# piotrkawa/audio-deepfake-adversarial-attacks

Measured on AMD Instinct MI355X. Metric: adversarial utterances/sec, PGD-40 LCNN+LFCC 4s@16kHz, higher is better.
Workload: dtype f32

## Files before the change

### audio_deepfake_adversarial_attacks_amd/_lib.py

```python
from __future__ import annotations

import ctypes
from pathlib import Path

import os

_LIB_PATH = Path(os.environ.get("ADVSTEP_LIB") or Path(__file__).resolve().parent / "libadvstep.so")
_lib = None

OK, EINVAL, EWORKSPACE, ELAUNCH, ENODEVICE = 0, 1, 2, 3, 4
ABI_VERSION = 3

_p, _i64, _f32, _f64, _u64, _sz = (ctypes.c_void_p, ctypes.c_int64, ctypes.c_float, ctypes.c_double,
                                   ctypes.c_uint64, ctypes.c_size_t)

SIGNATURES = {
    "advstep_abi_version": (ctypes.c_int, []),
    "advstep_status_string": (ctypes.c_char_p, [ctypes.c_int]),
    "advstep_device_count": (ctypes.c_int, []),
    "advstep_row_workspace_bytes": (_sz, [_i64, _i64]),
    "advstep_minmax_normalize_f32": (ctypes.c_int, [_p, _p, _p, _p, _i64, _i64, _p, _sz, _p]),
    "advstep_minmax_revert_f32": (ctypes.c_int, [_p, _p, _p, _p, _i64, _i64, _p]),
    "advstep_fgsm_step_f32": (ctypes.c_int, [_p, _p, _p, _i64, _f32, _f32, _f32, _p]),
    "advstep_pgd_linf_init_noise_f32": (ctypes.c_int, [_p, _p, _p, _i64, _f32, _f32, _p]),
# ... 8 lines not shown
    "advstep_cw_tanh_sqdist_f32": (ctypes.c_int, [_p, _p, _p, _p, _i64, _i64, _p, _sz, _p]),
    "advstep_cw_adam_step_f32": (ctypes.c_int, [_p, _p, _p, _p, _p, _i64, _i64, _f64, _f64, _f64, _f64, _p]),
    "advstep_cw_best_update_f32": (ctypes.c_int, [_p, _p, _p, _i64, _i64, _p]),
    "advstep_ce2_loss_grad_f32": (ctypes.c_int, [_p, _p, _p, _p, _i64, _f32, _p]),
    "advstep_mfm_sel_bytes": (_sz, [_i64, _i64, _i64]),
    "advstep_mfm_forward_f32": (ctypes.c_int, [_p, _p, _p, _p, _p, _p, _i64, _i64, _i64, _p]),
    "advstep_mfm_backward_f32": (ctypes.c_int, [_p, _p, _p, _p, _i64, _i64, _i64, _p]),
    "advstep_mfm_pool2_forward_f32": (ctypes.c_int, [_p, _p, _p, _p, _p, _p, _i64, _i64, _i64, _i64, _p]),
    "advstep_mfm_pool2_backward_f32": (ctypes.c_int, [_p, _p, _p, _p, _i64, _i64, _i64, _i64, _p]),
    "advstep_conv5_mfm_pool2_forward_f32": (ctypes.c_int, [_p, _p, _p, _p, _p, _i64, _i64, _i64, _i64, _p]),
    "advstep_conv5_mfm_pool2_backward_f32": (ctypes.c_int, [_p, _p, _p, _p, _i64, _i64, _i64, _i64, _p]),
    "advstep_conv1x1_mfm_supported": (ctypes.c_int, [_i64]),
    "advstep_conv1x1_mfm_sel_bytes": (_sz, [_i64, _i64, _i64]),
    "advstep_conv1x1_mfm_forward_f32": (ctypes.c_int, [_p, _p, _p, _p, _p, _p, _p, _i64, _i64, _i64, _i64, _p]),
    "advstep_conv1x1_mfm_backward_f32": (ctypes.c_int, [_p, _p, _p, _p, _p, _i64, _i64, _i64, _i64, _p]),
    "advstep_lstm_supported": (ctypes.c_int, [_i64]),
    "advstep_lstm_forward_f32": (ctypes.c_int, [_p, _p, _p, _p, _p, _i64, _i64, _i64, _i64, _p]),
    "advstep_lstm_backward_f32": (ctypes.c_int, [_p, _p, _p, _p, _p, _i64, _i64, _i64, _i64, _p]),
    "advstep_lstm_backward_bcast_f32": (ctypes.c_int, [_p, _p, _p, _p, _p, _i64, _i64, _i64, _i64, _p]),
    "advstep_lstm_backward_outer_f32": (ctypes.c_int, [_p, _p, _p, _p, _p, _p, _i64, _i64, _i64, _i64, _p]),
    "advstep_lcnn_tail_pack_f32": (ctypes.c_int, [_p, _p, _i64, _i64, _i64, _i64, _p]),
    "advstep_lcnn_tail_forward_f32": (ctypes.c_int, [_p, _p, _p, _p, _p, _i64, _i64, _i64, _p]),
    "advstep_lcnn_tail_unpack_add_f32": (ctypes.c_int, [_p, _p, _p, _i64, _i64, _i64, _i64, _p]),
    "advstep_lcnn_tail_unpack_add_outer_f32": (ctypes.c_int, [_p, _p, _p, _p, _i64, _i64, _i64, _i64, _p]),
    "advstep_gru_supported": (ctypes.c_int, [_i64]),
    "advstep_gru_forward_f32": (ctypes.c_int, [_p, _p, _p, _p, _p, _i64, _i64, _i64, _i64, _p]),
    "advstep_gru_backward_f32": (ctypes.c_int, [_p, _p, _p, _p, _p, _i64, _i64, _i64, _i64, _p]),
    "advstep_conv3x3_supported": (ctypes.c_int, [_i64, _i64]),
    "advstep_conv3x3_prepared_floats": (_sz, [_i64, _i64, ctypes.c_int]),
    "advstep_conv3x3_prepare_f32": (ctypes.c_int, [_p, _p, _p, _i64, _i64, ctypes.c_int, _p]),
# ... 146 lines not shown
```

### audio_deepfake_adversarial_attacks_amd/csrc/lcnn_conv1x1.hip

```cpp

#include <hip/hip_runtime.h>
#include <math.h>
#include <stdint.h>

#include "advstep_lcnn.h"
#include "advstep_common.h"

namespace {

constexpr int kBlock = 256;
constexpr int kPixPerBlock = 128;

typedef float f32x16 __attribute__((ext_vector_type(16)));

__device__ __forceinline__ int mfma_row(int r, int lane) { return (r & 3) + 8 * (r >> 2) + 4 * (lane >> 5); }

__host__ __device__ constexpr int sel_bit(int s) { return 16 * (s >> 4) + 2 * (s & 1) + 4 * ((s >> 2) & 3); }
__host__ __device__ constexpr int sel_half(int s) { return (s >> 1) & 1; }
inline int64_t sel_mask_bytes(int64_t C) { return C <= 32 ? 2 : 4; }

template <int CIN, int TILES, int MODE>
__global__ __launch_bounds__(kBlock) void conv1x1_mfm_forward_kernel(const float *__restrict__ x,
                                                                     const float *__restrict__ weight,
                                                                     const float *__restrict__ bias,
                                                                     const float *__restrict__ bn_mean,
                                                                     const float *__restrict__ bn_invstd,
                                                                     float *__restrict__ y, uint8_t *__restrict__ sel,
                                                                     int C, int64_t P, int64_t PW) {
    extern __shared__ __attribute__((aligned(16))) float w_s[];
    constexpr int CP = TILES * 32, PITCH = CIN + 1;
    constexpr uint32_t SELB = TILES == 1 ? 2u : 4u;
    float *par_s = w_s + 2 * CP * PITCH;
    constexpr int kWLoads = 2 * CP * CIN / kBlock;
    constexpr int kWBatch = kWLoads % 8 == 0 ? 8 : 12;
    static_assert((2 * CP * CIN) % kBlock == 0 && kWLoads % kWBatch == 0, "weight staging batches");
#pragma unroll
    for (int j0 = 0; j0 < kWLoads; j0 += kWBatch) {
        float wv[kWBatch];
#pragma unroll
        for (int j = 0; j < kWBatch; ++j) {
            const int i = threadIdx.x + (j0 + j) * kBlock, row = i / CIN, ci = i - row * CIN;
            const int half = row / CP, c = row - half * CP;
            wv[j] = weight[(half * C + (c < C ? c : 0)) * CIN + ci];
        }
#pragma unroll
        for (int j = 0; j < kWBatch; ++j) {
            const int i = threadIdx.x + (j0 + j) * kBlock, row = i / CIN, ci = i - row * CIN;
            const int c = row % CP;
            w_s[row * PITCH + ci] = c < C ? wv[j] : 0.0f;
        }
    }
    for (int c = threadIdx.x; c < CP; c += kBlock) {
        const bool live = c < C;
        par_s[c] = (bias && live) ? bias[c] : 0.0f;
        par_s[CP + c] = (bias && live) ? bias[c + C] : 0.0f;
        par_s[2 * CP + c] = (bn_mean && live) ? bn_mean[c] : 0.0f;
        par_s[3 * CP + c] = (bn_mean && live) ? bn_invstd[c] : 1.0f;
    }
    __syncthreads();

    const int64_t n = blockIdx.y;
    const int wave = threadIdx.x >> 6, lane = threadIdx.x & 63, li = lane & 31, lk = lane >> 5;
    const int64_t wave_p0 = ((int64_t)blockIdx.x * 4 + wave) * 32;
    if (wave_p0 >= P) return;
    const int64_t p = wave_p0 + li;
    const bool valid = p < P;
    const uint32_t Pb = (uint32_t)P * 4u;
    const __amdgpu_buffer_rsrc_t xr =
        __builtin_amdgcn_make_buffer_rsrc(const_cast<float *>(x + n * CIN * P), 0, (int)(CIN * Pb), 0x00020000);
    const __amdgpu_buffer_rsrc_t yr = __builtin_amdgcn_make_buffer_rsrc(y + n * (int64_t)C * P, 0, (int)(C * Pb), 0x00020000);
    const __amdgpu_buffer_rsrc_t sr =
        __builtin_amdgcn_make_buffer_rsrc(sel + n * PW * (int64_t)(64u * SELB), 0, (int)((uint32_t)PW * 64u * SELB), 0x00020000);
    constexpr uint32_t kOut = 0x80000000u;
    const uint32_t pb = (uint32_t)p * 4u;
    const uint32_t x_off = valid ? (uint32_t)lk * Pb + pb : kOut;
    const uint32_t y_off = valid ? 4u * (uint32_t)lk * Pb + pb : kOut;
    const uint32_t s_off = valid ? (uint32_t)(2 * li + lk) * SELB : kOut;
    const uint32_t s_tile = (uint32_t)(wave_p0 >> 5) * 64u * SELB;
    uint32_t mask = 0;
    float xb[CIN / 2];
#pragma unroll
    for (int s = 0; s < CIN / 2; ++s)
        xb[s] = __builtin_bit_cast(float, __builtin_amdgcn_raw_buffer_load_b32(xr, x_off, (uint32_t)(2 * s) * Pb, 0));

    constexpr bool FULL = MODE != 0;
    constexpr int kPairTiles = MODE == 2 ? TILES - 1 : TILES;
#pragma unroll
    for (int t = 0; t < kPairTiles; ++t) {
        f32x16 acc_a = {0}, acc_b = {0};
        const float *wa = w_s + (t * 32 + li) * PITCH + lk;
        const float *wb = wa + CP * PITCH;
#pragma unroll
        for (int s = 0; s < CIN / 2; ++s) {
            acc_a = __builtin_amdgcn_mfma_f32_32x32x2f32(wa[2 * s], xb[s], acc_a, 0, 0, 0);
            acc_b = __builtin_amdgcn_mfma_f32_32x32x2f32(wb[2 * s], xb[s], acc_b, 0, 0, 0);
        }
#pragma unroll
        for (int r = 0; r < 16; ++r) {
// ... 20 lines not shown
#pragma unroll
        for (int r = 0; r < 8; ++r) {
            const int c_lo = t * 32 + (r & 3) + 8 * (r >> 2);
            const int c = c_lo + 4 * lk;
            const float va = acc[r] + par_s[c], vb = acc[r + 8] + par_s[CP + c];
            const bool tb = mfm_takes_b(va, vb);
            mask |= tb ? (1u << (16 * t + r)) : 0u;
            const float v = ((tb ? vb : va) - par_s[2 * CP + c]) * par_s[3 * CP + c];
            __builtin_amdgcn_raw_buffer_store_b32(__builtin_bit_cast(uint32_t, v), yr, y_off, (uint32_t)c_lo * Pb, 0);
        }
    }
    if constexpr (SELB == 2) __builtin_amdgcn_raw_buffer_store_b16((uint16_t)mask, sr, s_off, s_tile, 0);
    else __builtin_amdgcn_raw_buffer_store_b32(mask, sr, s_off, s_tile, 0);
}

template <int CIN, int MT, int STEPS>
__global__ __launch_bounds__(kBlock) void conv1x1_mfm_backward_kernel(const float *__restrict__ gy,
                                                                      const uint8_t *__restrict__ sel,
                                                                      const float *__restrict__ weight,
                                                                      const float *__restrict__ gscale,
                                                                      float *__restrict__ gx, int C, int64_t P,
                                                                      int64_t PW) {
    extern __shared__ __attribute__((aligned(16))) float w_s[];
    constexpr int CW = MT * 32, PITCH = CW + 1;
    float *gs_s = w_s + 2 * C * PITCH;
    if constexpr (STEPS > 0) {
        constexpr int kRows = 4 * STEPS, kWLoads = kRows * CW / kBlock, kWBatch = kWLoads % 8 == 0 ? 8 : 12;
        static_assert((kRows * CW) % kBlock == 0 && kWLoads % kWBatch == 0, "weight staging batches");
#pragma unroll
        for (int j0 = 0; j0 < kWLoads; j0 += kWBatch) {
            float wv[kWBatch];
#pragma unroll
            for (int j = 0; j < kWBatch; ++j) {
                const int i = threadIdx.x + (j0 + j) * kBlock, row = i / CW, ci = i - row * CW;
                wv[j] = weight[row * CIN + (ci < CIN ? ci : 0)];
            }
#pragma unroll
            for (int j = 0; j < kWBatch; ++j) {
                const int i = threadIdx.x + (j0 + j) * kBlock, row = i / CW, ci = i - row * CW;
                w_s[row * PITCH + ci] = ci < CIN ? wv[j] : 0.0f;
            }
        }
    } else {
        for (int i = threadIdx.x; i < 2 * C * CW; i += kBlock) {
            const int row = i / CW, ci = i - row * CW;
            w_s[row * PITCH + ci] = ci < CIN ? weight[(int64_t)row * CIN + ci] : 0.0f;
        }
    }
    for (int c = threadIdx.x; c < C; c += kBlock) gs_s[c] = gscale ? gscale[c] : 1.0f;
    __syncthreads();

    const int64_t n = blockIdx.y;
    const int wave = threadIdx.x >> 6, lane = threadIdx.x & 63, li = lane & 31, lk = lane >> 5;
    const int64_t p = (int64_t)blockIdx.x * kPixPerBlock + wave * 32 + li;
    const bool valid = p < P;
    if ((int64_t)blockIdx.x * kPixPerBlock + wave * 32 >= P) return;

    const uint32_t Pb = (uint32_t)P * 4u;
    const bool wide = C > 32;
    const uint32_t pairb = wide ? 8u : 4u;
    const __amdgpu_buffer_rsrc_t gr =
        __builtin_amdgcn_make_buffer_rsrc(const_cast<float *>(gy + n * (int64_t)C * P), 0, (int)(C * Pb), 0x00020000);
    const __amdgpu_buffer_rsrc_t sr = __builtin_amdgcn_make_buffer_rsrc(
        const_cast<uint8_t *>(sel + n * PW * (int64_t)(32u * pairb)), 0, (int)((uint32_t)PW * 32u * pairb), 0x00020000);
    const __amdgpu_buffer_rsrc_t xr = __builtin_amdgcn_make_buffer_rsrc(gx + n * CIN * P, 0, (int)(CIN * Pb), 0x00020000);
    constexpr uint32_t kOut = 0x80000000u;
    const uint32_t pb = (uint32_t)p * 4u;
    const uint32_t g_off = valid ? (uint32_t)lk * Pb + pb : kOut;
    const uint32_t x_off = valid ? 4u * (uint32_t)lk * Pb + pb : kOut;
    const uint32_t s_off = valid ? (uint32_t)li * pairb : kOut;
    const uint32_t s_tile = (uint32_t)(((int64_t)blockIdx.x * kPixPerBlock + wave * 32) >> 5) * 32u * pairb;
    uint32_t m[2];
    if (wide) {
        m[0] = __builtin_amdgcn_raw_buffer_load_b32(sr, s_off, s_tile, 0) >> lk;
        m[1] = __builtin_amdgcn_raw_buffer_load_b32(sr, s_off + (valid ? 4u : 0u), s_tile, 0) >> lk;
    } else {
        const uint32_t both = __builtin_amdgcn_raw_buffer_load_b32(sr, s_off, s_tile, 0);
        m[0] = (both & 0xffffu) >> lk;
        m[1] = (both >> 16) >> lk;
    }
    f32x16 acc[MT];
#pragma unroll
    for (int m = 0; m < MT; ++m) acc[m] = (f32x16){0};
    if constexpr (STEPS > 0) {
        float g[STEPS];
#pragma unroll
        for (int s = 0; s < STEPS; ++s)
            g[s] = __builtin_bit_cast(float, __builtin_amdgcn_raw_buffer_load_b32(gr, g_off, (uint32_t)(2 * s) * Pb, 0));
#pragma unroll
        for (int s = 0; s < STEPS; ++s) {
            const int c = 2 * s + lk;
            const float gs = g[s] * gs_s[c];
            const bool tb = (m[sel_half(s)] >> sel_bit(s)) & 1u;
            const float ga = tb ? 0.0f : gs, gb = tb ? gs : 0.0f;
            const float *wa = w_s + c * PITCH + li;
            const float *wb = wa + C * PITCH;
#pragma unroll
            for (int m = 0; m < MT; ++m) {
                acc[m] = __builtin_amdgcn_mfma_f32_32x32x2f32(wa[32 * m], ga, acc[m], 0, 0, 0);
                acc[m] = __builtin_amdgcn_mfma_f32_32x32x2f32(wb[32 * m], gb, acc[m], 0, 0, 0);
            }
        }
    } else {
    const int steps = (C + 1) >> 1;
    for (int s = 0; s < steps; ++s) {
        const int c = 2 * s + lk;
        const bool live = c < C;
        const float g = live ? __builtin_bit_cast(float, __builtin_amdgcn_raw_buffer_load_b32(gr, g_off, (uint32_t)(2 * s) * Pb, 0)) *
                                   gs_s[c]
                             : 0.0f;
        const bool tb = live && ((m[sel_half(s)] >> sel_bit(s)) & 1u);
        const float ga = tb ? 0.0f : g, gb = tb ? g : 0.0f;
        const float *wa = w_s + (live ? c : 0) * PITCH + li;
        const float *wb = w_s + ((live ? c : 0) + C) * PITCH + li;
#pragma unroll
        for (int m = 0; m < MT; ++m) {
            acc[m] = __builtin_amdgcn_mfma_f32_32x32x2f32(live ? wa[32 * m] : 0.0f, ga, acc[m], 0, 0, 0);
            acc[m] = __builtin_amdgcn_mfma_f32_32x32x2f32(live ? wb[32 * m] : 0.0f, gb, acc[m], 0, 0, 0);
// ... 8 lines not shown
            static_assert(CIN % 8 == 0, "row pairs (ci, ci + 4) must be live or dead together");
            const float gv = acc[m][r];
            if (ci_lo < CIN)
                __builtin_amdgcn_raw_buffer_store_b32(__float_as_uint(gv), xr, x_off, (uint32_t)ci_lo * Pb, 0);
        }
    }
}

template <typename K>
void opt_in_lds(K kernel, size_t bytes) {
    if (bytes > 48 * 1024)
        (void)hipFuncSetAttribute(reinterpret_cast<const void *>(kernel), hipFuncAttributeMaxDynamicSharedMemorySize,
                                  (int)bytes);
}

template <int CIN, int TILES>
void launch_fwd(const float *x, const float *w, const float *b, const float *bn_mean, const float *bn_invstd, float *y,
                uint8_t *sel, int64_t N, int64_t C, int64_t P, hipStream_t st) {
    const size_t lds = (size_t)(2 * TILES * 32 * (CIN + 1) + 4 * TILES * 32) * sizeof(float);
    const dim3 grid((unsigned)ceil_div(P, kPixPerBlock), (unsigned)N);
    if (C == TILES * 32) {
        opt_in_lds(conv1x1_mfm_forward_kernel<CIN, TILES, 1>, lds);
        hipLaunchKernelGGL((conv1x1_mfm_forward_kernel<CIN, TILES, 1>), grid, dim3(kBlock), lds, st, x, w, b, bn_mean,
                           bn_invstd, y, sel, (int)C, P, ceil_div(P, 32));
    } else if (C == TILES * 32 - 16) {
        opt_in_lds(conv1x1_mfm_forward_kernel<CIN, TILES, 2>, lds);
        hipLaunchKernelGGL((conv1x1_mfm_forward_kernel<CIN, TILES, 2>), grid, dim3(kBlock), lds, st, x, w, b, bn_mean,
                           bn_invstd, y, sel, (int)C, P, ceil_div(P, 32));
    } else {
        opt_in_lds(conv1x1_mfm_forward_kernel<CIN, TILES, 0>, lds);
        hipLaunchKernelGGL((conv1x1_mfm_forward_kernel<CIN, TILES, 0>), grid, dim3(kBlock), lds, st, x, w, b, bn_mean,
                           bn_invstd, y, sel, (int)C, P, ceil_div(P, 32));
    }
}

template <int CIN, int MT, int STEPS>
void launch_bwd_steps(const float *gy, const uint8_t *sel, const float *w, const float *gscale, float *gx, int64_t N,
                      int64_t C, int64_t P, hipStream_t st) {
    const size_t lds = (size_t)(2 * C * (MT * 32 + 1) + C) * sizeof(float);
    opt_in_lds(conv1x1_mfm_backward_kernel<CIN, MT, STEPS>, lds);
    const dim3 grid((unsigned)ceil_div(P, kPixPerBlock), (unsigned)N);
    hipLaunchKernelGGL((conv1x1_mfm_backward_kernel<CIN, MT, STEPS>), grid, dim3(kBlock), lds, st, gy, sel, w, gscale, gx,
                       (int)C, P, ceil_div(P, 32));
}

template <int CIN, int MT>
void launch_bwd(const float *gy, const uint8_t *sel, const float *w, const float *gscale, float *gx, int64_t N, int64_t C,
                int64_t P, hipStream_t st) {
    if (C == CIN)
        launch_bwd_steps<CIN, MT, CIN / 2>(gy, sel, w, gscale, gx, N, C, P, st);
    else
        launch_bwd_steps<CIN, MT, 0>(gy, sel, w, gscale, gx, N, C, P, st);
}

}

extern "C" {

int advstep_conv1x1_mfm_supported(int64_t Cin) { return Cin == 32 || Cin == 48 || Cin == 64; }

size_t advstep_conv1x1_mfm_sel_bytes(int64_t N, int64_t C, int64_t P) {
    if (N <= 0 || C <= 0 || P <= 0) return 0;
    return (size_t)N * (size_t)ceil_div(P, 32) * 64u * (size_t)sel_mask_bytes(C);
}

int advstep_conv1x1_mfm_forward_f32(const float *x, const float *weight, const float *bias, const float *bn_mean,
                                    const float *bn_invstd, float *y, void *sel, int64_t N, int64_t Cin, int64_t C,
                                    int64_t P, advstep_stream_t stream) {
    ADVSTEP_REQUIRE(N >= 0 && C >= 0 && P >= 0 && advstep_conv1x1_mfm_supported(Cin));
    if (N == 0 || C == 0 || P == 0) return ADVSTEP_OK;
    ADVSTEP_REQUIRE(x && weight && y && sel && N <= kMaxGridY && C <= 64 && ((reinterpret_cast<uintptr_t>(sel) & 3u) == 0));
    ADVSTEP_REQUIRE((bn_mean == nullptr) == (bn_invstd == nullptr));
    auto *s32 = static_cast<uint8_t *>(sel);
    hipStream_t st = as_stream(stream);
    const bool two = C > 32;
    switch (Cin) {
        case 32:
            two ? launch_fwd<32, 2>(x, weight, bias, bn_mean, bn_invstd, y, s32, N, C, P, st)
                : launch_fwd<32, 1>(x, weight, bias, bn_mean, bn_invstd, y, s32, N, C, P, st);
            break;
        case 48:
            two ? launch_fwd<48, 2>(x, weight, bias, bn_mean, bn_invstd, y, s32, N, C, P, st)
                : launch_fwd<48, 1>(x, weight, bias, bn_mean, bn_invstd, y, s32, N, C, P, st);
            break;
        default:
            two ? launch_fwd<64, 2>(x, weight, bias, bn_mean, bn_invstd, y, s32, N, C, P, st)
                : launch_fwd<64, 1>(x, weight, bias, bn_mean, bn_invstd, y, s32, N, C, P, st);
            break;
    }
    return status_after_launch();
}

int advstep_conv1x1_mfm_backward_f32(const float *gy, const void *sel, const float *weight, const float *gscale, float *gx,
                                     int64_t N, int64_t Cin, int64_t C, int64_t P, advstep_stream_t stream) {
    ADVSTEP_REQUIRE(N >= 0 && C >= 0 && P >= 0 && advstep_conv1x1_mfm_supported(Cin));
    if (N == 0 || P == 0) return ADVSTEP_OK;
    ADVSTEP_REQUIRE(gx && N <= kMaxGridY && C <= 64);
    hipStream_t st = as_stream(stream);
    if (C == 0)
        return hipMemsetAsync(gx, 0, (size_t)N * Cin * P * sizeof(float), st) == hipSuccess ? ADVSTEP_OK : ADVSTEP_ELAUNCH;
    ADVSTEP_REQUIRE(gy && sel && weight);
    ADVSTEP_REQUIRE((reinterpret_cast<uintptr_t>(sel) & 3u) == 0);
    auto *s32 = static_cast<const uint8_t *>(sel);
    switch (Cin) {
        case 32: launch_bwd<32, 1>(gy, s32, weight, gscale, gx, N, C, P, st); break;
        case 48: launch_bwd<48, 2>(gy, s32, weight, gscale, gx, N, C, P, st); break;
        default: launch_bwd<64, 2>(gy, s32, weight, gscale, gx, N, C, P, st); break;
    }
    return status_after_launch();
}

}
```

### audio_deepfake_adversarial_attacks_amd/lcnn_ops.py

```python
from __future__ import annotations

from typing import Optional

import torch

from . import _lib
from .hip_ops import _Launch, _require, _stream


def _gemm(fn, a2d: torch.Tensor, b2d: torch.Tensor, *lead):
    with _Launch("rnn_projection_gemm", a2d.device, work=2.0 * a2d.shape[0] * a2d.shape[1] * b2d.shape[1]):
        return fn(*lead, a2d, b2d)


def _check_input(x: torch.Tensor, bias: Optional[torch.Tensor]):
    _require(x, "x")
    if x.dim() != 4 or x.shape[1] % 2 != 0:
        raise ValueError(f"expected a contiguous (N, 2C, H, W) tensor, got {tuple(x.shape)}")
    if bias is not None:
        _require(bias, "bias")
        if bias.numel() != x.shape[1]:
            raise ValueError(f"bias must have {x.shape[1]} entries, got {bias.numel()}")


# ... 106 lines not shown
        idx, weight = ctx.saved_tensors
        N, C, H, W = ctx.shape
        gy = gy.contiguous()
        gx = torch.empty((N, 1, H, W), dtype=gy.dtype, device=gy.device)
        with _Launch("conv5_mfm_pool2_backward", gy.device, work=12.5 * N * C * H * W, tensors=(gy, idx, gx)):
            st = _lib.load().advstep_conv5_mfm_pool2_backward_f32(gy.data_ptr(), idx.data_ptr(), weight.data_ptr(),
                                                                  gx.data_ptr(), N, C, H, W, _stream(gy.device))
        _lib.check(st, "advstep_conv5_mfm_pool2_backward_f32")
        return gx, None, None


def conv5_mfm_pool2(x: torch.Tensor, weight: torch.Tensor, bias: Optional[torch.Tensor] = None) -> torch.Tensor:
    return _Conv5MfmPool2.apply(x.contiguous(), weight.contiguous(), bias)


class _Conv1x1Mfm(torch.autograd.Function):

    @staticmethod
    def forward(ctx, x, weight, bias, bn):
        _require(x, "x"), _require(weight, "weight")
        if bias is not None:
            _require(bias, "bias")
        bn_mean, bn_invstd = _bn_ptrs(bn)
        if x.dim() != 4 or weight.dim() != 4 or tuple(weight.shape[2:]) != (1, 1) or weight.shape[1] != x.shape[1] \
                or weight.shape[0] % 2 != 0 or (bias is not None and bias.numel() != weight.shape[0]):
            raise ValueError(f"expected x (N, Cin, H, W), weight (2C, Cin, 1, 1), bias (2C); got {tuple(x.shape)}, "
                             f"{tuple(weight.shape)}")
        N, Cin, H, W = x.shape
        C, P = weight.shape[0] // 2, H * W
        lib = _lib.load()
        if not lib.advstep_conv1x1_mfm_supported(Cin):
            raise ValueError(f"conv1x1_mfm supports Cin in (32, 48, 64), got {Cin}")
        y = torch.empty((N, C, H, W), dtype=x.dtype, device=x.device)
        sel = torch.empty(max(lib.advstep_conv1x1_mfm_sel_bytes(N, C, P), 4), dtype=torch.uint8, device=x.device)
        with _Launch("conv1x1_mfm_forward", x.device, work=4.0 * N * Cin * C * P, tensors=(x, y, sel)):
            st = lib.advstep_conv1x1_mfm_forward_f32(x.data_ptr(), weight.data_ptr(),
                                                     bias.data_ptr() if bias is not None else None, bn_mean, bn_invstd,
                                                     y.data_ptr(), sel.data_ptr(), N, Cin, C, P, _stream(x.device))
        _lib.check(st, "advstep_conv1x1_mfm_forward_f32")
        ctx.save_for_backward(sel, weight, *([bn[1]] if bn is not None else []))
        ctx.shape = (N, Cin, C, H, W)
        return y

    @staticmethod
    def backward(ctx, gy):
        if ctx.needs_input_grad[1] or (len(ctx.needs_input_grad) > 2 and ctx.needs_input_grad[2]):
            raise RuntimeError("conv1x1_mfm provides the input gradient only; call it with frozen weights "
                               "(the model falls back to Conv2d + mfm otherwise)")
        sel, weight, *scale = ctx.saved_tensors
        N, Cin, C, H, W = ctx.shape
        gy = gy.contiguous()
        gx = torch.empty((N, Cin, H, W), dtype=gy.dtype, device=gy.device)
        with _Launch("conv1x1_mfm_backward", gy.device, work=4.0 * N * Cin * C * H * W, tensors=(gy, sel, gx)):
            st = _lib.load().advstep_conv1x1_mfm_backward_f32(gy.data_ptr(), sel.data_ptr(), weight.data_ptr(),
                                                              scale[0].data_ptr() if scale else None, gx.data_ptr(), N, Cin,
                                                              C, H * W, _stream(gy.device))
        _lib.check(st, "advstep_conv1x1_mfm_backward_f32")
        return gx, None, None, None


def conv1x1_mfm_supported(in_channels: int) -> bool:
    return bool(_lib.load().advstep_conv1x1_mfm_supported(in_channels))


def conv1x1_mfm(x: torch.Tensor, weight: torch.Tensor, bias: Optional[torch.Tensor] = None, bn=None) -> torch.Tensor:
    return _Conv1x1Mfm.apply(x.contiguous(), weight.contiguous(), bias, bn)



def _prepared_weights(weight: torch.Tensor, mode: int, gscale: Optional[torch.Tensor] = None) -> torch.Tensor:
    cache = getattr(weight, "_advstep_wino", None)
    if cache is None or cache[0] != (weight._version, weight.data_ptr()):
        cache = ((weight._version, weight.data_ptr()), {})
        try:
            weight._advstep_wino = cache
        except AttributeError:
            pass
    slot = (mode, None if gscale is None else (gscale.data_ptr(), gscale._version))
    U = cache[1].get(slot)
    if U is None:
        Cout, Cin = weight.shape[0], weight.shape[1]
# ... 326 lines not shown
```

### include/advstep_lcnn.h

```cpp
#ifndef ADVSTEP_LCNN_H_
#define ADVSTEP_LCNN_H_

#include <stddef.h>
#include <stdint.h>

#include "advstep.h"

#ifdef __cplusplus
extern "C" {
#endif

size_t advstep_mfm_sel_bytes(int64_t N, int64_t C, int64_t HW);

int advstep_mfm_forward_f32(const float *x, const float *bias, const float *bn_mean, const float *bn_invstd, float *y,
                            uint8_t *sel, int64_t N, int64_t C, int64_t HW, advstep_stream_t stream);

int advstep_mfm_backward_f32(const float *gy, const uint8_t *sel, const float *gscale, float *gx, int64_t N, int64_t C,
                             int64_t HW, advstep_stream_t stream);

int advstep_mfm_pool2_forward_f32(const float *x, const float *bias, const float *bn_mean, const float *bn_invstd,
                                  float *y, uint8_t *idx, int64_t N, int64_t C, int64_t H, int64_t W,
                                  advstep_stream_t stream);

int advstep_mfm_pool2_backward_f32(const float *gy, const uint8_t *idx, const float *gscale, float *gx, int64_t N,
// ... 1 lines not shown

int advstep_conv5_mfm_pool2_forward_f32(const float *x, const float *weight, const float *bias, float *y, uint8_t *idx,
                                        int64_t N, int64_t C, int64_t H, int64_t W, advstep_stream_t stream);

int advstep_conv5_mfm_pool2_backward_f32(const float *gy, const uint8_t *idx, const float *weight, float *gx, int64_t N,
                                         int64_t C, int64_t H, int64_t W, advstep_stream_t stream);

int advstep_conv1x1_mfm_supported(int64_t Cin);
size_t advstep_conv1x1_mfm_sel_bytes(int64_t N, int64_t C, int64_t P);
int advstep_conv1x1_mfm_forward_f32(const float *x, const float *weight, const float *bias, const float *bn_mean,
                                    const float *bn_invstd, float *y, void *sel, int64_t N, int64_t Cin, int64_t C,
                                    int64_t P, advstep_stream_t stream);

int advstep_conv1x1_mfm_backward_f32(const float *gy, const void *sel, const float *weight, const float *gscale,
                                     float *gx, int64_t N, int64_t Cin, int64_t C, int64_t P, advstep_stream_t stream);

int advstep_conv3x3_supported(int64_t Cin, int64_t Cout);
size_t advstep_conv3x3_prepared_floats(int64_t Cin, int64_t Cout, int mode);
int advstep_conv3x3_prepare_f32(const float *weight, const float *gscale, float *U, int64_t Cin, int64_t Cout, int mode,
                                advstep_stream_t stream);

int advstep_conv3x3_mfm_pool2_forward_f32(const float *x, const float *U, const float *bias, const float *bn_mean,
                                          const float *bn_invstd, float *y, uint8_t *idx, int64_t N, int64_t Cin,
                                          int64_t C, int64_t H, int64_t W, advstep_stream_t stream);

size_t advstep_conv3x3_mfm_sel_bytes(int64_t N, int64_t C, int64_t H, int64_t W);
int advstep_conv3x3_mfm_forward_f32(const float *x, const float *U, const float *bias, const float *bn_mean,
                                    const float *bn_invstd, float *y, uint8_t *sel, int64_t N, int64_t Cin, int64_t C,
                                    int64_t H, int64_t W, advstep_stream_t stream);
int advstep_conv3x3_mfm_backward_f32(const float *gy, const uint8_t *sel, const float *gscale, float *gout, int64_t N,
// ... 38 lines not shown
```

Measured before the change: 2040.

## Prepare padded conv1x1 weight images and stream them into LDS asynchronously

Adds a one-time prepare step that packs conv1x1 weights, bias, BN params and grad scales into a padded LDS-ready image. The image is cached on the frozen weight tensor. The forward and backward kernels then copy that image with global_load_lds DMA, which overlaps with their activation loads and replaces per-block strided weight staging through registers. The trade-offs are a host-side cache keyed on tensor version and pointer, extra template variants, and early-exit wave returns being dropped so every wave reaches the barrier.

After: 2048, median of 6. Within noise of the previous version (+0.4%).

```diff
diff --git a/audio_deepfake_adversarial_attacks_amd/_lib.py b/audio_deepfake_adversarial_attacks_amd/_lib.py
--- a/audio_deepfake_adversarial_attacks_amd/_lib.py
+++ b/audio_deepfake_adversarial_attacks_amd/_lib.py
@@ -46,6 +46,11 @@
     "advstep_conv1x1_mfm_sel_bytes": (_sz, [_i64, _i64, _i64]),
     "advstep_conv1x1_mfm_forward_f32": (ctypes.c_int, [_p, _p, _p, _p, _p, _p, _p, _i64, _i64, _i64, _i64, _p]),
     "advstep_conv1x1_mfm_backward_f32": (ctypes.c_int, [_p, _p, _p, _p, _p, _i64, _i64, _i64, _i64, _p]),
+    "advstep_conv1x1_mfm_prepared_floats": (_sz, [_i64, _i64, ctypes.c_int]),
+    "advstep_conv1x1_mfm_prepared_preferred": (ctypes.c_int, [_i64, _i64, ctypes.c_int]),
+    "advstep_conv1x1_mfm_prepare_f32": (ctypes.c_int, [_p, _p, _p, _p, _p, _i64, _i64, ctypes.c_int, _p]),
+    "advstep_conv1x1_mfm_forward_prepared_f32": (ctypes.c_int, [_p, _p, _p, _p, _i64, _i64, _i64, _i64, _p]),
+    "advstep_conv1x1_mfm_backward_prepared_f32": (ctypes.c_int, [_p, _p, _p, _p, _i64, _i64, _i64, _i64, _p]),
     "advstep_lstm_supported": (ctypes.c_int, [_i64]),
     "advstep_lstm_forward_f32": (ctypes.c_int, [_p, _p, _p, _p, _p, _i64, _i64, _i64, _i64, _p]),
     "advstep_lstm_backward_f32": (ctypes.c_int, [_p, _p, _p, _p, _p, _i64, _i64, _i64, _i64, _p]),
diff --git a/audio_deepfake_adversarial_attacks_amd/csrc/lcnn_conv1x1.hip b/audio_deepfake_adversarial_attacks_amd/csrc/lcnn_conv1x1.hip
--- a/audio_deepfake_adversarial_attacks_amd/csrc/lcnn_conv1x1.hip
+++ b/audio_deepfake_adversarial_attacks_amd/csrc/lcnn_conv1x1.hip
@@ -19,7 +19,78 @@
 __host__ __device__ constexpr int sel_half(int s) { return (s >> 1) & 1; }
 inline int64_t sel_mask_bytes(int64_t C) { return C <= 32 ? 2 : 4; }
 
-template <int CIN, int TILES, int MODE>
+__host__ __device__ constexpr int fwd_image_floats(int CIN, int TILES) { return 2 * TILES * 32 * (CIN + 1) + 4 * TILES * 32; }
+__host__ __device__ constexpr int bwd_image_floats(int C, int MT) { return (2 * C * (32 * MT + 1) + C + 3) & ~3; }
+__host__ __device__ constexpr int image_lds_bytes(int floats) { return ((floats / 4 + 63) & ~63) * 16; }
+
+template <int N4>
+__device__ __forceinline__ void image_to_lds(const float *__restrict__ image, float *lds, int n4_runtime) {
+    const float4 *src = reinterpret_cast<const float4 *>(image);
+    float4 *dst = reinterpret_cast<float4 *>(lds);
+    const int n4 = N4 > 0 ? N4 : n4_runtime;
+    const int w64 = __builtin_amdgcn_readfirstlane((int)(threadIdx.x >> 6) << 6), lane = threadIdx.x & 63;
+    if constexpr (N4 > 0) {
+#pragma unroll
+        for (int i = 0; i < (N4 + kBlock - 1) / kBlock; ++i) {
+            const int base = w64 + i * kBlock;
+            if (i * kBlock + kBlock - 64 < N4 || base < N4)
+                __builtin_amdgcn_global_load_lds((const __attribute__((address_space(1))) void *)(src + min(base + lane, N4 - 1)),
+                                                 (__attribute__((address_space(3))) void *)(dst + base), 16, 0, 0);
+        }
+    } else {
+        for (int base = w64; base < n4; base += kBlock)
+            __builtin_amdgcn_global_load_lds((const __attribute__((address_space(1))) void *)(src + min(base + lane, n4 - 1)),
+                                             (__attribute__((address_space(3))) void *)(dst + base), 16, 0, 0);
+    }
+    __builtin_amdgcn_sched_barrier(0);
+}
+template <int LATER>
+__device__ __forceinline__ void image_landed_barrier() {
+    static_assert(LATER >= 0 && LATER < 64, "vmcnt is a 6-bit counter");
+    __builtin_amdgcn_s_waitcnt((LATER & 15) | 0x0F70 | ((LATER >> 4) << 14));
+    __builtin_amdgcn_s_barrier();
+}
+
+__global__ __launch_bounds__(kBlock) void conv1x1_prepare_forward_kernel(const float *__restrict__ weight,
+                                                                         const float *__restrict__ bias,
+                                                                         const float *__restrict__ bn_mean,
+                                                                         const float *__restrict__ bn_invstd,
+                                                                         float *__restrict__ image, int CIN, int C, int CP) {
+    const int PITCH = CIN + 1, nw = 2 * CP * PITCH, n = nw + 4 * CP;
+    for (int i = blockIdx.x * kBlock + threadIdx.x; i < n; i += gridDim.x * kBlock) {
+        float v;
+        if (i < nw) {
+            const int row = i / PITCH, ci = i - row * PITCH, half = row / CP, c = row - half * CP;
+            v = (c < C && ci < CIN) ? weight[(half * C + c) * CIN + ci] : 0.0f;
+        } else {
+            const int j = i - nw, k = j / CP, c = j - k * CP;
+            const bool live = c < C;
+            if (k < 2) v = (bias && live) ? bias[c + k * C] : 0.0f;
+            else if (k == 2) v = (bn_mean && live) ? bn_mean[c] : 0.0f;
+            else v = (bn_mean && live) ? bn_invstd[c] : 1.0f;
+        }
+        image[i] = v;
+    }
+}
+
+__global__ __launch_bounds__(kBlock) void conv1x1_prepare_backward_kernel(const float *__restrict__ weight,
+                                                                          const float *__restrict__ gscale,
+                                                                          float *__restrict__ image, int CIN, int C, int CW,
+                                                                          int n) {
+    const int PITCH = CW + 1, nw = 2 * C * PITCH;
+    for (int i = blockIdx.x * kBlock + threadIdx.x; i < n; i += gridDim.x * kBlock) {
+        float v = 0.0f;
+        if (i < nw) {
+            const int row = i / PITCH, ci = i - row * PITCH;
+            v = ci < CIN ? weight[row * CIN + ci] : 0.0f;
+        } else if (i < nw + C) {
+            v = gscale ? gscale[i - nw] : 1.0f;
+        }
+        image[i] = v;
+    }
+}
+
+template <int CIN, int TILES, int MODE, bool PREP>
 __global__ __launch_bounds__(kBlock) void conv1x1_mfm_forward_kernel(const float *__restrict__ x,
                                                                      const float *__restrict__ weight,
                                                                      const float *__restrict__ bias,
@@ -34,6 +105,7 @@
     constexpr int kWLoads = 2 * CP * CIN / kBlock;
     constexpr int kWBatch = kWLoads % 8 == 0 ? 8 : 12;
     static_assert((2 * CP * CIN) % kBlock == 0 && kWLoads % kWBatch == 0, "weight staging batches");
+    if constexpr (!PREP) {
 #pragma unroll
     for (int j0 = 0; j0 < kWLoads; j0 += kWBatch) {
         float wv[kWBatch];
@@ -58,11 +130,16 @@
         par_s[3 * CP + c] = (bn_mean && live) ? bn_invstd[c] : 1.0f;
     }
     __syncthreads();
+    } else {
+        static_assert(fwd_image_floats(CIN, TILES) % 4 == 0, "the image is a whole number of float4");
+        image_to_lds<fwd_image_floats(CIN, TILES) / 4>(weight, w_s, 0);
+    }
 
     const int64_t n = blockIdx.y;
-    const int wave = threadIdx.x >> 6, lane = threadIdx.x & 63, li = lane & 31, lk = lane >> 5;
+    const int wave = PREP ? __builtin_amdgcn_readfirstlane((int)(threadIdx.x >> 6)) : (int)(threadIdx.x >> 6);
+    const int lane = threadIdx.x & 63, li = lane & 31, lk = lane >> 5;
     const int64_t wave_p0 = ((int64_t)blockIdx.x * 4 + wave) * 32;
-    if (wave_p0 >= P) return;
+    if (!PREP && wave_p0 >= P) return;
     const int64_t p = wave_p0 + li;
     const bool valid = p < P;
     const uint32_t Pb = (uint32_t)P * 4u;
@@ -82,6 +159,7 @@
 #pragma unroll
     for (int s = 0; s < CIN / 2; ++s)
         xb[s] = __builtin_bit_cast(float, __builtin_amdgcn_raw_buffer_load_b32(xr, x_off, (uint32_t)(2 * s) * Pb, 0));
+    if constexpr (PREP) image_landed_barrier<CIN / 2>();
 
     constexpr bool FULL = MODE != 0;
     constexpr int kPairTiles = MODE == 2 ? TILES - 1 : TILES;
@@ -132,7 +210,7 @@
     else __builtin_amdgcn_raw_buffer_store_b32(mask, sr, s_off, s_tile, 0);
 }
 
-template <int CIN, int MT, int STEPS>
+template <int CIN, int MT, int STEPS, bool PREP>
 __global__ __launch_bounds__(kBlock) void conv1x1_mfm_backward_kernel(const float *__restrict__ gy,
                                                                       const uint8_t *__restrict__ sel,
                                                                       const float *__restrict__ weight,
@@ -142,7 +220,10 @@
     extern __shared__ __attribute__((aligned(16))) float w_s[];
     constexpr int CW = MT * 32, PITCH = CW + 1;
     float *gs_s = w_s + 2 * C * PITCH;
-    if constexpr (STEPS > 0) {
+    if constexpr (PREP) {
+        if constexpr (STEPS > 0) image_to_lds<bwd_image_floats(2 * STEPS, MT) / 4>(weight, w_s, 0);
+        else image_to_lds<0>(weight, w_s, bwd_image_floats(C, MT) / 4);
+    } else if constexpr (STEPS > 0) {
         constexpr int kRows = 4 * STEPS, kWLoads = kRows * CW / kBlock, kWBatch = kWLoads % 8 == 0 ? 8 : 12;
         static_assert((kRows * CW) % kBlock == 0 && kWLoads % kWBatch == 0, "weight staging batches");
 #pragma unroll
@@ -165,17 +246,20 @@
             w_s[row * PITCH + ci] = ci < CIN ? weight[(int64_t)row * CIN + ci] : 0.0f;
         }
     }
+    if constexpr (!PREP) {
     for (int c = threadIdx.x; c < C; c += kBlock) gs_s[c] = gscale ? gscale[c] : 1.0f;
     __syncthreads();
+    }
 
     const int64_t n = blockIdx.y;
-    const int wave = threadIdx.x >> 6, lane = threadIdx.x & 63, li = lane & 31, lk = lane >> 5;
+    const int wave = PREP ? __builtin_amdgcn_readfirstlane((int)(threadIdx.x >> 6)) : (int)(threadIdx.x >> 6);
+    const int lane = threadIdx.x & 63, li = lane & 31, lk = lane >> 5;
     const int64_t p = (int64_t)blockIdx.x * kPixPerBlock + wave * 32 + li;
     const bool valid = p < P;
-    if ((int64_t)blockIdx.x * kPixPerBlock + wave * 32 >= P) return;
+    if (!PREP && (int64_t)blockIdx.x * kPixPerBlock + wave * 32 >= P) return;
 
     const uint32_t Pb = (uint32_t)P * 4u;
-    const bool wide = C > 32;
+    const bool wide = (PREP && STEPS > 0) ? STEPS > 16 : C > 32;
     const uint32_t pairb = wide ? 8u : 4u;
     const __amdgpu_buffer_rsrc_t gr =
         __builtin_amdgcn_make_buffer_rsrc(const_cast<float *>(gy + n * (int64_t)C * P), 0, (int)(C * Pb), 0x00020000);
@@ -205,6 +289,7 @@
 #pragma unroll
         for (int s = 0; s < STEPS; ++s)
             g[s] = __builtin_bit_cast(float, __builtin_amdgcn_raw_buffer_load_b32(gr, g_off, (uint32_t)(2 * s) * Pb, 0));
+        if constexpr (PREP) image_landed_barrier<STEPS + (STEPS > 16 ? 2 : 1)>();
 #pragma unroll
         for (int s = 0; s < STEPS; ++s) {
             const int c = 2 * s + lk;
@@ -220,6 +305,7 @@
             }
         }
     } else {
+    if constexpr (PREP) image_landed_barrier<0>();
     const int steps = (C + 1) >> 1;
     for (int s = 0; s < steps; ++s) {
         const int c = 2 * s + lk;
@@ -258,44 +344,75 @@
                                   (int)bytes);
 }
 
-template <int CIN, int TILES>
+template <int CIN, int TILES, bool PREP>
 void launch_fwd(const float *x, const float *w, const float *b, const float *bn_mean, const float *bn_invstd, float *y,
                 uint8_t *sel, int64_t N, int64_t C, int64_t P, hipStream_t st) {
-    const size_t lds = (size_t)(2 * TILES * 32 * (CIN + 1) + 4 * TILES * 32) * sizeof(float);
+    const size_t lds = PREP ? (size_t)image_lds_bytes(fwd_image_floats(CIN, TILES))
+                            : (size_t)(2 * TILES * 32 * (CIN + 1) + 4 * TILES * 32) * sizeof(float);
     const dim3 grid((unsigned)ceil_div(P, kPixPerBlock), (unsigned)N);
     if (C == TILES * 32) {
-        opt_in_lds(conv1x1_mfm_forward_kernel<CIN, TILES, 1>, lds);
-        hipLaunchKernelGGL((conv1x1_mfm_forward_kernel<CIN, TILES, 1>), grid, dim3(kBlock), lds, st, x, w, b, bn_mean,
+        opt_in_lds(conv1x1_mfm_forward_kernel<CIN, TILES, 1, PREP>, lds);
+        hipLaunchKernelGGL((conv1x1_mfm_forward_kernel<CIN, TILES, 1, PREP>), grid, dim3(kBlock), lds, st, x, w, b, bn_mean,
                            bn_invstd, y, sel, (int)C, P, ceil_div(P, 32));
     } else if (C == TILES * 32 - 16) {
-        opt_in_lds(conv1x1_mfm_forward_kernel<CIN, TILES, 2>, lds);
-        hipLaunchKernelGGL((conv1x1_mfm_forward_kernel<CIN, TILES, 2>), grid, dim3(kBlock), lds, st, x, w, b, bn_mean,
+        opt_in_lds(conv1x1_mfm_forward_kernel<CIN, TILES, 2, PREP>, lds);
+        hipLaunchKernelGGL((conv1x1_mfm_forward_kernel<CIN, TILES, 2, PREP>), grid, dim3(kBlock), lds, st, x, w, b, bn_mean,
                            bn_invstd, y, sel, (int)C, P, ceil_div(P, 32));
     } else {
-        opt_in_lds(conv1x1_mfm_forward_kernel<CIN, TILES, 0>, lds);
-        hipLaunchKernelGGL((conv1x1_mfm_forward_kernel<CIN, TILES, 0>), grid, dim3(kBlock), lds, st, x, w, b, bn_mean,
+        opt_in_lds(conv1x1_mfm_forward_kernel<CIN, TILES, 0, PREP>, lds);
+        hipLaunchKernelGGL((conv1x1_mfm_forward_kernel<CIN, TILES, 0, PREP>), grid, dim3(kBlock), lds, st, x, w, b, bn_mean,
                            bn_invstd, y, sel, (int)C, P, ceil_div(P, 32));
     }
 }
 
-template <int CIN, int MT, int STEPS>
+template <int CIN, bool PREP>
+void launch_fwd_tiles(const float *x, const float *w, const float *b, const float *bn_mean, const float *bn_invstd, float *y,
+                      uint8_t *sel, int64_t N, int64_t C, int64_t P, hipStream_t st) {
+    C > 32 ? launch_fwd<CIN, 2, PREP>(x, w, b, bn_mean, bn_invstd, y, sel, N, C, P, st)
+           : launch_fwd<CIN, 1, PREP>(x, w, b, bn_mean, bn_invstd, y, sel, N, C, P, st);
+}
+
+template <bool PREP>
+void launch_fwd_cin(const float *x, const float *w, const float *b, const float *bn_mean, const float *bn_invstd, float *y,
+                    uint8_t *sel, int64_t N, int64_t Cin, int64_t C, int64_t P, hipStream_t st) {
+    switch (Cin) {
+        case 32: launch_fwd_tiles<32, PREP>(x, w, b, bn_mean, bn_invstd, y, sel, N, C, P, st); break;
+        case 48: launch_fwd_tiles<48, PREP>(x, w, b, bn_mean, bn_invstd, y, sel, N, C, P, st); break;
+        default: launch_fwd_tiles<64, PREP>(x, w, b, bn_mean, bn_invstd, y, sel, N, C, P, st); break;
+    }
+}
+
+template <int CIN, int MT, int STEPS, bool PREP>
 void launch_bwd_steps(const float *gy, const uint8_t *sel, const float *w, const float *gscale, float *gx, int64_t N,
                       int64_t C, int64_t P, hipStream_t st) {
-    const size_t lds = (size_t)(2 * C * (MT * 32 + 1) + C) * sizeof(float);
-    opt_in_lds(conv1x1_mfm_backward_kernel<CIN, MT, STEPS>, lds);
+    const size_t lds = PREP ? (size_t)image_lds_bytes(bwd_image_floats((int)C, MT))
+                            : (size_t)(2 * C * (MT * 32 + 1) + C) * sizeof(float);
+    opt_in_lds(conv1x1_mfm_backward_kernel<CIN, MT, STEPS, PREP>, lds);
     const dim3 grid((unsigned)ceil_div(P, kPixPerBlock), (unsigned)N);
-    hipLaunchKernelGGL((conv1x1_mfm_backward_kernel<CIN, MT, STEPS>), grid, dim3(kBlock), lds, st, gy, sel, w, gscale, gx,
-                       (int)C, P, ceil_div(P, 32));
-}
-
-template <int CIN, int MT>
+    hipLaunchKernelGGL((conv1x1_mfm_backward_kernel<CIN, MT, STEPS, PREP>), grid, dim3(kBlock), lds, st, gy, sel, w, gscale,
+                       gx, (int)C, P, ceil_div(P, 32));
+}
+
+template <int CIN, int MT, bool PREP>
 void launch_bwd(const float *gy, const uint8_t *sel, const float *w, const float *gscale, float *gx, int64_t N, int64_t C,
                 int64_t P, hipStream_t st) {
     if (C == CIN)
-        launch_bwd_steps<CIN, MT, CIN / 2>(gy, sel, w, gscale, gx, N, C, P, st);
+        launch_bwd_steps<CIN, MT, CIN / 2, PREP>(gy, sel, w, gscale, gx, N, C, P, st);
     else
-        launch_bwd_steps<CIN, MT, 0>(gy, sel, w, gscale, gx, N, C, P, st);
-}
+        launch_bwd_steps<CIN, MT, 0, PREP>(gy, sel, w, gscale, gx, N, C, P, st);
+}
+
+template <bool PREP>
+void launch_bwd_cin(const float *gy, const uint8_t *sel, const float *w, const float *gscale, float *gx, int64_t N,
+                    int64_t Cin, int64_t C, int64_t P, hipStream_t st) {
+    switch (Cin) {
+        case 32: launch_bwd<32, 1, PREP>(gy, sel, w, gscale, gx, N, C, P, st); break;
+        case 48: launch_bwd<48, 2, PREP>(gy, sel, w, gscale, gx, N, C, P, st); break;
+        default: launch_bwd<64, 2, PREP>(gy, sel, w, gscale, gx, N, C, P, st); break;
+    }
+}
+
+inline int mt_of(int64_t Cin) { return Cin > 32 ? 2 : 1; }
 
 }
 
@@ -315,23 +432,7 @@
     if (N == 0 || C == 0 || P == 0) return ADVSTEP_OK;
     ADVSTEP_REQUIRE(x && weight && y && sel && N <= kMaxGridY && C <= 64 && ((reinterpret_cast<uintptr_t>(sel) & 3u) == 0));
     ADVSTEP_REQUIRE((bn_mean == nullptr) == (bn_invstd == nullptr));
-    auto *s32 = static_cast<uint8_t *>(sel);
-    hipStream_t st = as_stream(stream);
-    const bool two = C > 32;
-    switch (Cin) {
-        case 32:
-            two ? launch_fwd<32, 2>(x, weight, bias, bn_mean, bn_invstd, y, s32, N, C, P, st)
-                : launch_fwd<32, 1>(x, weight, bias, bn_mean, bn_invstd, y, s32, N, C, P, st);
-            break;
-        case 48:
-            two ? launch_fwd<48, 2>(x, weight, bias, bn_mean, bn_invstd, y, s32, N, C, P, st)
-                : launch_fwd<48, 1>(x, weight, bias, bn_mean, bn_invstd, y, s32, N, C, P, st);
-            break;
-        default:
-            two ? launch_fwd<64, 2>(x, weight, bias, bn_mean, bn_invstd, y, s32, N, C, P, st)
-                : launch_fwd<64, 1>(x, weight, bias, bn_mean, bn_invstd, y, s32, N, C, P, st);
-            break;
-    }
+    launch_fwd_cin<false>(x, weight, bias, bn_mean, bn_invstd, y, static_cast<uint8_t *>(sel), N, Cin, C, P, as_stream(stream));
     return status_after_launch();
 }
 
@@ -345,13 +446,62 @@
         return hipMemsetAsync(gx, 0, (size_t)N * Cin * P * sizeof(float), st) == hipSuccess ? ADVSTEP_OK : ADVSTEP_ELAUNCH;
     ADVSTEP_REQUIRE(gy && sel && weight);
     ADVSTEP_REQUIRE((reinterpret_cast<uintptr_t>(sel) & 3u) == 0);
-    auto *s32 = static_cast<const uint8_t *>(sel);
-    switch (Cin) {
-        case 32: launch_bwd<32, 1>(gy, s32, weight, gscale, gx, N, C, P, st); break;
-        case 48: launch_bwd<48, 2>(gy, s32, weight, gscale, gx, N, C, P, st); break;
-        default: launch_bwd<64, 2>(gy, s32, weight, gscale, gx, N, C, P, st); break;
-    }
+    launch_bwd_cin<false>(gy, static_cast<const uint8_t *>(sel), weight, gscale, gx, N, Cin, C, P, st);
     return status_after_launch();
 }
 
-}
+size_t advstep_conv1x1_mfm_prepared_floats(int64_t Cin, int64_t C, int direction) {
+    if (!advstep_conv1x1_mfm_supported(Cin) || C <= 0 || C > 64 || (direction != 0 && direction != 1)) return 0;
+    return direction == 0 ? (size_t)fwd_image_floats((int)Cin, C > 32 ? 2 : 1) : (size_t)bwd_image_floats((int)C, mt_of(Cin));
+}
+
+int advstep_conv1x1_mfm_prepared_preferred(int64_t Cin, int64_t C, int direction) {
+    if (advstep_conv1x1_mfm_prepared_floats(Cin, C, direction) == 0) return 0;
+    if (Cin == 48 && C == 48) return 1;
+    return Cin == 32 && C == 32 && direction == 1;
+}
+
+int advstep_conv1x1_mfm_prepare_f32(const float *weight, const float *bias, const float *bn_mean, const float *scale,
+                                    float *image, int64_t Cin, int64_t C, int direction, advstep_stream_t stream) {
+    ADVSTEP_REQUIRE(C >= 0 && C <= 64 && advstep_conv1x1_mfm_supported(Cin) && (direction == 0 || direction == 1));
+    if (C == 0) return ADVSTEP_OK;
+    ADVSTEP_REQUIRE(weight && image && aligned16(image));
+    const int n = (int)advstep_conv1x1_mfm_prepared_floats(Cin, C, direction);
+    const dim3 grid((unsigned)ceil_div(n, 4 * kBlock));
+    if (direction == 0) {
+        ADVSTEP_REQUIRE((bn_mean == nullptr) == (scale == nullptr));
+        hipLaunchKernelGGL(conv1x1_prepare_forward_kernel, grid, dim3(kBlock), 0, as_stream(stream), weight, bias, bn_mean, scale,
+                           image, (int)Cin, (int)C, C > 32 ? 64 : 32);
+    } else {
+        ADVSTEP_REQUIRE(bias == nullptr && bn_mean == nullptr);
+        hipLaunchKernelGGL(conv1x1_prepare_backward_kernel, grid, dim3(kBlock), 0, as_stream(stream), weight, scale, image,
+                           (int)Cin, (int)C, 32 * mt_of(Cin), n);
+    }
+    return status_after_launch();
+}
+
+int advstep_conv1x1_mfm_forward_prepared_f32(const float *x, const float *image, float *y, void *sel, int64_t N, int64_t Cin,
+                                             int64_t C, int64_t P, advstep_stream_t stream) {
+    ADVSTEP_REQUIRE(N >= 0 && C >= 0 && P >= 0 && advstep_conv1x1_mfm_supported(Cin));
+    if (N == 0 || C == 0 || P == 0) return ADVSTEP_OK;
+    ADVSTEP_REQUIRE(x && image && aligned16(image) && y && sel && N <= kMaxGridY && C <= 64 &&
+                    ((reinterpret_cast<uintptr_t>(sel) & 3u) == 0));
+    launch_fwd_cin<true>(x, image, nullptr, nullptr, nullptr, y, static_cast<uint8_t *>(sel), N, Cin, C, P, as_stream(stream));
+    return status_after_launch();
+}
+
+int advstep_conv1x1_mfm_backward_prepared_f32(const float *gy, const void *sel, const float *image, float *gx, int64_t N,
+                                              int64_t Cin, int64_t C, int64_t P, advstep_stream_t stream) {
+    ADVSTEP_REQUIRE(N >= 0 && C >= 0 && P >= 0 && advstep_conv1x1_mfm_supported(Cin));
+    if (N == 0 || P == 0) return ADVSTEP_OK;
+    ADVSTEP_REQUIRE(gx && N <= kMaxGridY && C <= 64);
+    hipStream_t st = as_stream(stream);
+    if (C == 0)
+        return hipMemsetAsync(gx, 0, (size_t)N * Cin * P * sizeof(float), st) == hipSuccess ? ADVSTEP_OK : ADVSTEP_ELAUNCH;
+    ADVSTEP_REQUIRE(gy && sel && image && aligned16(image));
+    ADVSTEP_REQUIRE((reinterpret_cast<uintptr_t>(sel) & 3u) == 0);
+    launch_bwd_cin<true>(gy, static_cast<const uint8_t *>(sel), image, nullptr, gx, N, Cin, C, P, st);
+    return status_after_launch();
+}
+
+}
diff --git a/audio_deepfake_adversarial_attacks_amd/lcnn_ops.py b/audio_deepfake_adversarial_attacks_amd/lcnn_ops.py
--- a/audio_deepfake_adversarial_attacks_amd/lcnn_ops.py
+++ b/audio_deepfake_adversarial_attacks_amd/lcnn_ops.py
@@ -1,5 +1,6 @@
 from __future__ import annotations
 
+import os
 from typing import Optional
 
 import torch
@@ -144,31 +145,72 @@
     return _Conv5MfmPool2.apply(x.contiguous(), weight.contiguous(), bias)
 
 
+def _conv1x1_prepared_enabled() -> bool:
+    return os.environ.get("ADVSTEP_CONV1X1_PREPARED", "1") != "0"
+
+
+def _conv1x1_image(weight: torch.Tensor, direction: int, bias: Optional[torch.Tensor], bn) -> Optional[torch.Tensor]:
+    if not _conv1x1_prepared_enabled():
+        return None
+    C, Cin = weight.shape[0] // 2, weight.shape[1]
+    lib = _lib.load()
+    if not lib.advstep_conv1x1_mfm_prepared_preferred(Cin, C, direction):
+        return None
+    key = (weight._version, weight.data_ptr())
+    cache = getattr(weight, "_advstep_conv1x1", None)
+    if cache is None or cache[0] != key:
+        cache = (key, {})
+        try:
+            weight._advstep_conv1x1 = cache
+        except AttributeError:
+            return None
+    if direction == 0:
+        others = (bias,) + (tuple(bn) if bn is not None else (None, None))
+    else:
+        others = (None, None, bn[1] if bn is not None else None)
+    slot = (direction,) + tuple(None if t is None else (t.data_ptr(), t._version) for t in others)
+    hit = cache[1].get(slot)
+    if hit is not None:
+        return hit[0]
+    image = torch.empty(lib.advstep_conv1x1_mfm_prepared_floats(Cin, C, direction), dtype=torch.float32,
+                        device=weight.device)
+    with _Launch("conv1x1_prepare", weight.device):
+        st = lib.advstep_conv1x1_mfm_prepare_f32(weight.data_ptr(), *(None if t is None else t.data_ptr() for t in others),
+                                                 image.data_ptr(), Cin, C, direction, _stream(weight.device))
+    _lib.check(st, "advstep_conv1x1_mfm_prepare_f32")
+    if len(cache[1]) >= 8:
+        cache[1].clear()
+    cache[1][slot] = (image, others)
+    return image
+
+
 class _Conv1x1Mfm(torch.autograd.Function):
 
     @staticmethod
-    def forward(ctx, x, weight, bias, bn):
+    def forward(ctx, x, weight, bias, bn, image, image_grad):
         _require(x, "x"), _require(weight, "weight")
         if bias is not None:
             _require(bias, "bias")
         bn_mean, bn_invstd = _bn_ptrs(bn)
-        if x.dim() != 4 or weight.dim() != 4 or tuple(weight.shape[2:]) != (1, 1) or weight.shape[1] != x.shape[1] \
-                or weight.shape[0] % 2 != 0 or (bias is not None and bias.numel() != weight.shape[0]):
-            raise ValueError(f"expected x (N, Cin, H, W), weight (2C, Cin, 1, 1), bias (2C); got {tuple(x.shape)}, "
-                             f"{tuple(weight.shape)}")
         N, Cin, H, W = x.shape
         C, P = weight.shape[0] // 2, H * W
         lib = _lib.load()
-        if not lib.advstep_conv1x1_mfm_supported(Cin):
-            raise ValueError(f"conv1x1_mfm supports Cin in (32, 48, 64), got {Cin}")
         y = torch.empty((N, C, H, W), dtype=x.dtype, device=x.device)
         sel = torch.empty(max(lib.advstep_conv1x1_mfm_sel_bytes(N, C, P), 4), dtype=torch.uint8, device=x.device)
         with _Launch("conv1x1_mfm_forward", x.device, work=4.0 * N * Cin * C * P, tensors=(x, y, sel)):
-            st = lib.advstep_conv1x1_mfm_forward_f32(x.data_ptr(), weight.data_ptr(),
-                                                     bias.data_ptr() if bias is not None else None, bn_mean, bn_invstd,
-                                                     y.data_ptr(), sel.data_ptr(), N, Cin, C, P, _stream(x.device))
+            if image is not None:
+                st = lib.advstep_conv1x1_mfm_forward_prepared_f32(x.data_ptr(), image.data_ptr(), y.data_ptr(),
+                                                                  sel.data_ptr(), N, Cin, C, P, _stream(x.device))
+            else:
+                st = lib.advstep_conv1x1_mfm_forward_f32(x.data_ptr(), weight.data_ptr(),
+                                                         bias.data_ptr() if bias is not None else None, bn_mean, bn_invstd,
+                                                         y.data_ptr(), sel.data_ptr(), N, Cin, C, P, _stream(x.device))
         _lib.check(st, "advstep_conv1x1_mfm_forward_f32")
-        ctx.save_for_backward(sel, weight, *([bn[1]] if bn is not None else []))
+        ctx.prepared = image_grad is not None
+        if ctx.prepared:
+            ctx.save_for_backward(sel, image_grad)
+        else:
+            ctx.save_for_backward(sel, weight, *([bn[1]] if bn is not None else []))
         ctx.shape = (N, Cin, C, H, W)
         return y
 
@@ -182,11 +224,16 @@
         gy = gy.contiguous()
         gx = torch.empty((N, Cin, H, W), dtype=gy.dtype, device=gy.device)
         with _Launch("conv1x1_mfm_backward", gy.device, work=4.0 * N * Cin * C * H * W, tensors=(gy, sel, gx)):
-            st = _lib.load().advstep_conv1x1_mfm_backward_f32(gy.data_ptr(), sel.data_ptr(), weight.data_ptr(),
-                                                              scale[0].data_ptr() if scale else None, gx.data_ptr(), N, Cin,
-                                                              C, H * W, _stream(gy.device))
+            if ctx.prepared:
+                st = _lib.load().advstep_conv1x1_mfm_backward_prepared_f32(gy.data_ptr(), sel.data_ptr(), weight.data_ptr(),
+                                                                           gx.data_ptr(), N, Cin, C, H * W,
+                                                                           _stream(gy.device))
+            else:
+                st = _lib.load().advstep_conv1x1_mfm_backward_f32(gy.data_ptr(), sel.data_ptr(), weight.data_ptr(),
+                                                                  scale[0].data_ptr() if scale else None, gx.data_ptr(), N,
+                                                                  Cin, C, H * W, _stream(gy.device))
         _lib.check(st, "advstep_conv1x1_mfm_backward_f32")
-        return gx, None, None, None
+        return gx, None, None, None, None, None
 
 
 def conv1x1_mfm_supported(in_channels: int) -> bool:
@@ -194,7 +241,22 @@
 
 
 def conv1x1_mfm(x: torch.Tensor, weight: torch.Tensor, bias: Optional[torch.Tensor] = None, bn=None) -> torch.Tensor:
-    return _Conv1x1Mfm.apply(x.contiguous(), weight.contiguous(), bias, bn)
+    _require(x, "x"), _require(weight, "weight")
+    if bias is not None:
+        _require(bias, "bias")
+    _bn_ptrs(bn)
+    if x.dim() != 4 or weight.dim() != 4 or tuple(weight.shape[2:]) != (1, 1) or weight.shape[1] != x.shape[1] \
+            or weight.shape[0] % 2 != 0 or (bias is not None and bias.numel() != weight.shape[0]):
+        raise ValueError(f"expected x (N, Cin, H, W), weight (2C, Cin, 1, 1), bias (2C); got {tuple(x.shape)}, "
+                         f"{tuple(weight.shape)}")
+    if not conv1x1_mfm_supported(x.shape[1]):
+        raise ValueError(f"conv1x1_mfm supports Cin in (32, 48, 64), got {x.shape[1]}")
+    weight = weight.contiguous()
+    image = image_grad = None
+    if 0 < weight.shape[0] // 2 <= 64 and not weight.requires_grad:
+        image = _conv1x1_image(weight, 0, bias, bn)
+        image_grad = _conv1x1_image(weight, 1, None, bn) if x.requires_grad else None
+    return _Conv1x1Mfm.apply(x.contiguous(), weight, bias, bn, image, image_grad)
 
 
 
diff --git a/include/advstep_lcnn.h b/include/advstep_lcnn.h
--- a/include/advstep_lcnn.h
+++ b/include/advstep_lcnn.h
@@ -39,6 +39,15 @@
 
 int advstep_conv1x1_mfm_backward_f32(const float *gy, const void *sel, const float *weight, const float *gscale,
                                      float *gx, int64_t N, int64_t Cin, int64_t C, int64_t P, advstep_stream_t stream);
+
+size_t advstep_conv1x1_mfm_prepared_floats(int64_t Cin, int64_t C, int direction);
+int advstep_conv1x1_mfm_prepared_preferred(int64_t Cin, int64_t C, int direction);
+int advstep_conv1x1_mfm_prepare_f32(const float *weight, const float *bias, const float *bn_mean, const float *scale,
+                                    float *image, int64_t Cin, int64_t C, int direction, advstep_stream_t stream);
+int advstep_conv1x1_mfm_forward_prepared_f32(const float *x, const float *image, float *y, void *sel, int64_t N,
+                                             int64_t Cin, int64_t C, int64_t P, advstep_stream_t stream);
+int advstep_conv1x1_mfm_backward_prepared_f32(const float *gy, const void *sel, const float *image, float *gx, int64_t N,
+                                              int64_t Cin, int64_t C, int64_t P, advstep_stream_t stream);
 
 int advstep_conv3x3_supported(int64_t Cin, int64_t Cout);
 size_t advstep_conv3x3_prepared_floats(int64_t Cin, int64_t Cout, int mode);
```
